# microsoft/M3P

Measured on AMD Instinct MI355X. Metric: pre-train samples/sec (whole node), 12L/768d seq=128+36, higher is better.
Workload: dtype bf16; 1 GPU; cfg2: 12L/768d/12h, 36 regions + 128 tokens, V=250002, 19 MLM targets/seq + ITM BCE, dropout 0.10, adam_inverse_sqrt + clip 5; per_gpu_batch=256, global_batch=256, seq_len=164, parallelism=dp1, prewarm_steps=36

## Files before the change

m3p_amd/csrc/embed.hip:

```cpp
#include "common.hpp"
#include <hip/amd_detail/amd_hip_unsafe_atomics.h>

namespace {

constexpr int EMB_BWD_BLOCKS = 512;

constexpr float kEps = 1e-12f;

template <int NI>
__device__ __forceinline__ void row_ln(const f32x4 (&v)[NI], int nchunk, int lane, float inv_d, float& mu, float& rs) {
  float s = 0.f;
#pragma unroll
  for (int i = 0; i < NI; ++i) s += (v[i][0] + v[i][1]) + (v[i][2] + v[i][3]);
  mu = wave_sum(s) * inv_d;
  float q = 0.f;
#pragma unroll
  for (int i = 0; i < NI; ++i) {
    if (lane + 64 * i < nchunk) {
      const f32x4 t = v[i] - mu;
      q += (t[0] * t[0] + t[1] * t[1]) + (t[2] * t[2] + t[3] * t[3]);
    }
  }
  rs = 1.0f / sqrtf(wave_sum(q) * inv_d + kEps);
}

struct EmbedFwdArgs {
  const int64_t* tok;
  const bf16* emb;
  const float* pos;
  const bf16* img_proj;
  const float* loc;
  const float* w_loc;
  const float* b_loc;
  const float* g_img; const float* be_img;
  const float* g_emb; const float* be_emb;
  const int32_t* totlen;
  bf16* h;
  bf16* z;
  float* mean_emb; float* rstd_emb;
  bf16* e;
  float* mean_img; float* rstd_img;
  int B, T, R, d;
  uint32_t seed_img, seed_emb, thresh24; float inv_keep;
  bf16* img_rows; int img_mode;
};

template <int NI>
__global__ __launch_bounds__(256) void embed_fwd_kernel(EmbedFwdArgs a) {
  const int lane = threadIdx.x & 63;
  const int wave = (blockIdx.x * blockDim.x + threadIdx.x) >> 6;
  const int nwaves = (gridDim.x * blockDim.x) >> 6;
  const int S = a.R + a.T, d = a.d, nchunk = d >> 2;
  const float inv_d = 1.0f / (float)d;
  for (int m = wave; m < a.B * S; m += nwaves) {
    const int b = m / S, s = m - b * S;
    const float mk = (a.img_mode == 1 || s < a.totlen[b]) ? 1.f : 0.f;
    f32x4 v[NI];
    if (s < a.R && a.img_mode == 2) {
#pragma unroll
      for (int i = 0; i < NI; ++i) {
        const int c = lane + 64 * i;
        v[i] = f32x4{0.f, 0.f, 0.f, 0.f};
        if (c < nchunk) v[i] = Vec4<bf16>::load(a.img_rows + ((size_t)b * a.R + s) * d + 4 * c);
      }
    } else if (s < a.R) {
      const int ri = s * a.B + b;
      float lc[5];
#pragma unroll
      for (int k = 0; k < 5; ++k) lc[k] = a.loc[(size_t)ri * 5 + k];
#pragma unroll
      for (int i = 0; i < NI; ++i) {
        const int c = lane + 64 * i;
        v[i] = f32x4{0.f, 0.f, 0.f, 0.f};
        if (c < nchunk) {
          f32x4 t = Vec4<bf16>::load(a.img_proj + (size_t)ri * d + 4 * c) + Vec4<float>::load(a.b_loc + 4 * c);
#pragma unroll
          for (int j = 0; j < 4; ++j) {
            const float* w = a.w_loc + (size_t)(4 * c + j) * 5;
            t[j] += w[0] * lc[0] + w[1] * lc[1] + w[2] * lc[2] + w[3] * lc[3] + w[4] * lc[4];
          }
          t = round_bf16(t);
          Vec4<bf16>::store(a.e + (size_t)ri * d + 4 * c, t);
          v[i] = t;
        }
      }
      float mu, rs;
      row_ln<NI>(v, nchunk, lane, inv_d, mu, rs);
      if (lane == 0) { a.mean_img[ri] = mu; a.rstd_img[ri] = rs; }
#pragma unroll
      for (int i = 0; i < NI; ++i) {
        const int c = lane + 64 * i;
        if (c < nchunk) {
          f32x4 o = (v[i] - mu) * rs * Vec4<float>::load(a.g_img + 4 * c) + Vec4<float>::load(a.be_img + 4 * c);
          if (a.thresh24) {
            const uint32_t base = (uint32_t)ri * (uint32_t)d + 4u * c;
            { bool kp[4]; m3p_keep_even<4>(base, a.seed_img, a.thresh24, kp);
#pragma unroll
          for (int j = 0; j < 4; ++j) o[j] = kp[j] ? o[j] * a.inv_keep : 0.f; }
          }
          v[i] = o;
          if (a.img_mode == 1) Vec4<bf16>::store(a.img_rows + ((size_t)b * a.R + s) * d + 4 * c, o);
        }
      }
      if (a.img_mode == 1) continue;
    } else {
      const int64_t id = a.tok[(size_t)(s - a.R) * a.B + b];
#pragma unroll
      for (int i = 0; i < NI; ++i) {
        const int c = lane + 64 * i;
        v[i] = f32x4{0.f, 0.f, 0.f, 0.f};
        if (c < nchunk) v[i] = Vec4<bf16>::load(a.emb + (size_t)id * d + 4 * c);
      }
    }
#pragma unroll
    for (int i = 0; i < NI; ++i) {
      const int c = lane + 64 * i;
      if (c < nchunk) {
        const f32x4 t = round_bf16((v[i] + Vec4<float>::load(a.pos + (size_t)s * d + 4 * c)) * mk);
        Vec4<bf16>::store(a.z + (size_t)m * d + 4 * c, t);
        v[i] = t;
      }
    }
    float mu, rs;
    row_ln<NI>(v, nchunk, lane, inv_d, mu, rs);
    if (lane == 0) { a.mean_emb[m] = mu; a.rstd_emb[m] = rs; }
#pragma unroll
    for (int i = 0; i < NI; ++i) {
      const int c = lane + 64 * i;
      if (c < nchunk) {
        f32x4 o = (v[i] - mu) * rs * Vec4<float>::load(a.g_emb + 4 * c) + Vec4<float>::load(a.be_emb + 4 * c);
        if (a.thresh24) {
          const uint32_t base = (uint32_t)m * (uint32_t)d + 4u * c;
          { bool kp[4]; m3p_keep_even<4>(base, a.seed_emb, a.thresh24, kp);
#pragma unroll
          for (int j = 0; j < 4; ++j) o[j] = kp[j] ? o[j] * a.inv_keep : 0.f; }
        }
        Vec4<bf16>::store(a.h + (size_t)m * d + 4 * c, o);
      }
    }
  }
}

struct EmbedBwdArgs {
  const bf16* dh;
  const bf16* z; const float* mean_emb; const float* rstd_emb; const float* g_emb;
  const bf16* e; const float* mean_img; const float* rstd_img; const float* g_img;
  const int64_t* tok; const int32_t* totlen; const float* loc;
  bf16* dz;
  bf16* de;
  float* d_g_emb; float* d_be_emb; float* d_pos;
  float* d_emb;
  bf16* d_tok_rows;
  float* d_g_img; float* d_be_img; float* d_b_img; float* d_b_loc; float* d_w_loc;
  int B, T, R, d, pad_index, bsplit;
  uint32_t seed_img, seed_emb, thresh24; float inv_keep;
};

template <int NI>
__device__ __forceinline__ void block_reduce_atomic(float (*red)[NI * 256], const f32x4 (&acc)[NI], float* out, int d,
                                                    int lane, int wib) {
#pragma unroll
  for (int i = 0; i < NI; ++i)
#pragma unroll
    for (int j = 0; j < 4; ++j) red[wib][4 * (lane + 64 * i) + j] = acc[i][j];
  __syncthreads();
  for (int c = threadIdx.x; c < d; c += blockDim.x)
    unsafeAtomicAdd(out + c, (red[0][c] + red[1][c]) + (red[2][c] + red[3][c]));
  __syncthreads();
}

template <int NI>
__global__ __launch_bounds__(256) void embed_bwd_rows_kernel(EmbedBwdArgs a) {
  __shared__ float red[4][NI * 256];
  const int lane = threadIdx.x & 63, wib = threadIdx.x >> 6;
  const int S = a.R + a.T, d = a.d, nchunk = d >> 2;
  const float inv_d = 1.0f / (float)d;
  const int s = blockIdx.x / a.bsplit, part = blockIdx.x - s * a.bsplit;
  f32x4 g[NI], acc_g[NI], acc_b[NI], acc_p[NI];
#pragma unroll
  for (int i = 0; i < NI; ++i) {
    const int c = lane + 64 * i;
    g[i] = f32x4{0.f, 0.f, 0.f, 0.f};
    if (c < nchunk) g[i] = Vec4<float>::load(a.g_emb + 4 * c);
    acc_g[i] = acc_b[i] = acc_p[i] = f32x4{0.f, 0.f, 0.f, 0.f};
  }
  for (int b = part * 4 + wib; b < a.B; b += 4 * a.bsplit) {
    const size_t m = (size_t)b * S + s;
    const float mu = a.mean_emb[m], rs = a.rstd_emb[m];
    const float mk = (s < a.totlen[b]) ? 1.f : 0.f;
    f32x4 dy[NI], xh[NI];
    float s1 = 0.f, s2 = 0.f;
#pragma unroll
    for (int i = 0; i < NI; ++i) {
      const int c = lane + 64 * i;
      dy[i] = xh[i] = f32x4{0.f, 0.f, 0.f, 0.f};
      if (c < nchunk) {
        dy[i] = Vec4<bf16>::load(a.dh + m * d + 4 * c);
        if (a.thresh24) {
          const uint32_t base = (uint32_t)m * (uint32_t)d + 4u * c;
          { bool kp[4]; m3p_keep_even<4>(base, a.seed_emb, a.thresh24, kp);
#pragma unroll
          for (int j = 0; j < 4; ++j) dy[i][j] = kp[j] ? dy[i][j] * a.inv_keep : 0.f; }
        }
        xh[i] = (Vec4<bf16>::load(a.z + m * d + 4 * c) - mu) * rs;
        const f32x4 gd = dy[i] * g[i];
        s1 += (gd[0] + gd[1]) + (gd[2] + gd[3]);
        const f32x4 gx = gd * xh[i];
        s2 += (gx[0] + gx[1]) + (gx[2] + gx[3]);
        acc_g[i] += dy[i] * xh[i];
        acc_b[i] += dy[i];
      }
    }
    const float c1 = wave_sum(s1) * inv_d, c2 = wave_sum(s2) * inv_d;
    int64_t id = -1;
    if (s >= a.R) id = a.tok[(size_t)(s - a.R) * a.B + b];
#pragma unroll
    for (int i = 0; i < NI; ++i) {
      const int c = lane + 64 * i;
      if (c < nchunk) {
        const f32x4 o = (dy[i] * g[i] - c1 - xh[i] * c2) * rs * mk;
        acc_p[i] += o;
        if (s < a.R) {
          Vec4<bf16>::store(a.dz + m * d + 4 * c, o);
        } else {
          *reinterpret_cast<f32x4*>(&red[wib][4 * c]) = o;
        }
      }
    }
    if (s >= a.R && a.d_tok_rows) {
      const bool live = id != a.pad_index && mk != 0.f;
      bf16* dr = a.d_tok_rows + ((size_t)(s - a.R) * a.B + b) * d;
#pragma unroll
      for (int i = 0; i < NI; ++i) {
        const int c = lane + 64 * i;
        if (c < nchunk) {
          f32x4 o = *reinterpret_cast<const f32x4*>(&red[wib][4 * c]);
          if (!live) o = f32x4{0.f, 0.f, 0.f, 0.f};
// ... 19 lines not shown
__global__ __launch_bounds__(256) void embed_bwd_img_kernel(EmbedBwdArgs a) {
  __shared__ float red[4][NI * 256];
  const int lane = threadIdx.x & 63, wib = threadIdx.x >> 6;
  const int S = a.R + a.T, d = a.d, nchunk = d >> 2;
  const float inv_d = 1.0f / (float)d;
  const int r = blockIdx.x / a.bsplit, part = blockIdx.x - r * a.bsplit;
  f32x4 g[NI], acc_g[NI], acc_b[NI], acc_e[NI], acc_w[5][NI];
#pragma unroll
  for (int i = 0; i < NI; ++i) {
    const int c = lane + 64 * i;
    g[i] = f32x4{0.f, 0.f, 0.f, 0.f};
    if (c < nchunk) g[i] = Vec4<float>::load(a.g_img + 4 * c);
    acc_g[i] = acc_b[i] = acc_e[i] = f32x4{0.f, 0.f, 0.f, 0.f};
#pragma unroll
    for (int k = 0; k < 5; ++k) acc_w[k][i] = f32x4{0.f, 0.f, 0.f, 0.f};
  }
  for (int b = part * 4 + wib; b < a.B; b += 4 * a.bsplit) {
    const size_t m = (size_t)b * S + r;
    const size_t ri = (size_t)r * a.B + b;
    const float mu = a.mean_img[ri], rs = a.rstd_img[ri];
    float lc[5];
#pragma unroll
    for (int k = 0; k < 5; ++k) lc[k] = a.loc[ri * 5 + k];
    f32x4 dy[NI], xh[NI];
    float s1 = 0.f, s2 = 0.f;
#pragma unroll
    for (int i = 0; i < NI; ++i) {
      const int c = lane + 64 * i;
      dy[i] = xh[i] = f32x4{0.f, 0.f, 0.f, 0.f};
      if (c < nchunk) {
        dy[i] = Vec4<bf16>::load(a.dz + m * d + 4 * c);
        if (a.thresh24) {
          const uint32_t base = (uint32_t)ri * (uint32_t)d + 4u * c;
          { bool kp[4]; m3p_keep_even<4>(base, a.seed_img, a.thresh24, kp);
#pragma unroll
          for (int j = 0; j < 4; ++j) dy[i][j] = kp[j] ? dy[i][j] * a.inv_keep : 0.f; }
        }
        xh[i] = (Vec4<bf16>::load(a.e + ri * d + 4 * c) - mu) * rs;
        const f32x4 gd = dy[i] * g[i];
        s1 += (gd[0] + gd[1]) + (gd[2] + gd[3]);
        const f32x4 gx = gd * xh[i];
        s2 += (gx[0] + gx[1]) + (gx[2] + gx[3]);
        acc_g[i] += dy[i] * xh[i];
        acc_b[i] += dy[i];
      }
    }
    const float c1 = wave_sum(s1) * inv_d, c2 = wave_sum(s2) * inv_d;
#pragma unroll
    for (int i = 0; i < NI; ++i) {
      const int c = lane + 64 * i;
      if (c < nchunk) {
        const f32x4 ob = round_bf16((dy[i] * g[i] - c1 - xh[i] * c2) * rs);
        Vec4<bf16>::store(a.de + ri * d + 4 * c, ob);
        acc_e[i] += ob;
#pragma unroll
        for (int k = 0; k < 5; ++k) acc_w[k][i] += ob * lc[k];
      }
    }
  }
  block_reduce_atomic<NI>(red, acc_g, a.d_g_img, d, lane, wib);
  block_reduce_atomic<NI>(red, acc_b, a.d_be_img, d, lane, wib);
#pragma unroll
  for (int i = 0; i < NI; ++i)
#pragma unroll
    for (int j = 0; j < 4; ++j) red[wib][4 * (lane + 64 * i) + j] = acc_e[i][j];
  __syncthreads();
  for (int c = threadIdx.x; c < d; c += blockDim.x) {
    const float v = (red[0][c] + red[1][c]) + (red[2][c] + red[3][c]);
    unsafeAtomicAdd(a.d_b_img + c, v);
    unsafeAtomicAdd(a.d_b_loc + c, v);
  }
  __syncthreads();
#pragma unroll
  for (int k = 0; k < 5; ++k) {
#pragma unroll
    for (int i = 0; i < NI; ++i)
#pragma unroll
      for (int j = 0; j < 4; ++j) red[wib][4 * (lane + 64 * i) + j] = acc_w[k][i][j];
    __syncthreads();
    for (int c = threadIdx.x; c < d; c += blockDim.x)
      unsafeAtomicAdd(a.d_w_loc + (size_t)c * 5 + k, (red[0][c] + red[1][c]) + (red[2][c] + red[3][c]));
    __syncthreads();
  }
}

__global__ __launch_bounds__(256) void cast_f32_bf16_kernel(const float* __restrict__ src, bf16* __restrict__ dst, size_t n4) {
  for (size_t i = (size_t)blockIdx.x * blockDim.x + threadIdx.x; i < n4; i += (size_t)gridDim.x * blockDim.x)
    Vec4<bf16>::store(dst + 4 * i, Vec4<float>::load(src + 4 * i));
}

inline int ni_of(int d) { return (d + 255) / 256; }

int launch_embed_fwd(const EmbedFwdArgs& a, void* stream);
}

extern "C" {

int m3p_cast_f32_bf16(const float* src, void* dst, long long n, void* stream) {
  if (n <= 0 || (n % 4) != 0 || ((uintptr_t)src & 15) || ((uintptr_t)dst & 7)) return M3P_EINVAL;
  const size_t n4 = (size_t)n / 4;
  const int blocks = (int)((n4 + 255) / 256 < 4096 ? (n4 + 255) / 256 : 4096);
  hipLaunchKernelGGL(cast_f32_bf16_kernel, dim3(blocks), dim3(256), 0, (hipStream_t)stream, src, (bf16*)dst, n4);
  M3P_CHECK_LAUNCH();
  return M3P_OK;
}

int m3p_embed_assemble_fwd(const int64_t* tok, const void* emb_bf16, const float* pos, const void* img_proj,
                           const float* loc, const float* w_loc, const float* b_loc, const float* g_img,
                           const float* be_img, const float* g_emb, const float* be_emb, const int32_t* totlen,
                           void* h, void* z, float* mean_emb, float* rstd_emb, void* e, float* mean_img,
                           float* rstd_img, int B, int T, int R, int d, uint32_t seed_img, uint32_t seed_emb,
                           uint32_t thresh24, float inv_keep, const void* img_rows, void* stream) {
  if (B <= 0 || T < 0 || R < 0 || d <= 0 || (d % 4) != 0 || d > 1024) return M3P_EINVAL;
  if (img_rows && ((uintptr_t)img_rows & 7)) return M3P_EINVAL;
  EmbedFwdArgs a = {tok, (const bf16*)emb_bf16, pos, (const bf16*)img_proj, loc, w_loc, b_loc, g_img, be_img, g_emb, be_emb,
                    totlen, (bf16*)h, (bf16*)z, mean_emb, rstd_emb, (bf16*)e, mean_img, rstd_img, B, T, R, d,
                    seed_img, seed_emb, thresh24, inv_keep, (bf16*)const_cast<void*>(img_rows), img_rows ? 2 : 0};
  return launch_embed_fwd(a, stream);
}

int m3p_embed_image_rows_fwd(const void* img_proj, const float* loc, const float* w_loc, const float* b_loc,
                             const float* g_img, const float* be_img, void* e, float* mean_img, float* rstd_img,
                             void* img_rows, int B, int R, int d, uint32_t seed_img, uint32_t thresh24, float inv_keep,
                             void* stream) {
  if (B <= 0 || R <= 0 || d <= 0 || (d % 4) != 0 || d > 1024 || !img_rows || ((uintptr_t)img_rows & 7)) return M3P_EINVAL;
  EmbedFwdArgs a = {nullptr, nullptr, nullptr, (const bf16*)img_proj, loc, w_loc, b_loc, g_img, be_img, nullptr, nullptr,
                    nullptr, nullptr, nullptr, nullptr, nullptr, (bf16*)e, mean_img, rstd_img, B, 0, R, d,
                    seed_img, 0u, thresh24, inv_keep, (bf16*)img_rows, 1};
  return launch_embed_fwd(a, stream);
}

}

namespace {
int launch_embed_fwd(const EmbedFwdArgs& a, void* stream) {
  const int B = a.B, T = a.T, R = a.R, d = a.d;
  const int rows = B * (R + T);
  const int blocks = (rows + 3) / 4 < 4096 ? (rows + 3) / 4 : 4096;
  hipStream_t st = (hipStream_t)stream;
  switch (ni_of(d)) {
    case 1: hipLaunchKernelGGL(embed_fwd_kernel<1>, dim3(blocks), dim3(256), 0, st, a); break;
    case 2: hipLaunchKernelGGL(embed_fwd_kernel<2>, dim3(blocks), dim3(256), 0, st, a); break;
    case 3: hipLaunchKernelGGL(embed_fwd_kernel<3>, dim3(blocks), dim3(256), 0, st, a); break;
    default: hipLaunchKernelGGL(embed_fwd_kernel<4>, dim3(blocks), dim3(256), 0, st, a); break;
  }
  M3P_CHECK_LAUNCH();
  return M3P_OK;
}
}

extern "C" {

int m3p_embed_assemble_bwd(const void* dh, const void* z, const float* mean_emb, const float* rstd_emb,
                           const float* g_emb, const void* e, const float* mean_img, const float* rstd_img,
                           const float* g_img, const int64_t* tok, const int32_t* totlen, const float* loc,
                           void* dz_scratch, void* de, float* d_g_emb, float* d_be_emb, float* d_pos, float* d_emb,
                           void* d_tok_rows, float* d_g_img, float* d_be_img, float* d_b_img, float* d_b_loc, float* d_w_loc,
                           int B, int T, int R, int d, int pad_index, uint32_t seed_img, uint32_t seed_emb,
                           uint32_t thresh24, float inv_keep, int phase, void* stream) {
  if (B <= 0 || T < 0 || R < 0 || d <= 0 || (d % 4) != 0 || d > 1024 || phase < 0 || phase > 2) return M3P_EINVAL;
  int bsplit = 1;
  while (bsplit < 16 && (R + T) * bsplit < EMB_BWD_BLOCKS && B / (4 * bsplit) >= 8) bsplit *= 2;
  EmbedBwdArgs a = {(const bf16*)dh, (const bf16*)z, mean_emb, rstd_emb, g_emb, (const bf16*)e, mean_img, rstd_img, g_img,
                    tok, totlen, loc, (bf16*)dz_scratch, (bf16*)de, d_g_emb, d_be_emb, d_pos, d_emb,
                    (bf16*)d_tok_rows, d_g_img, d_be_img, d_b_img, d_b_loc, d_w_loc, B, T, R, d, pad_index, bsplit,
                    seed_img, seed_emb, thresh24, inv_keep};
  hipStream_t st = (hipStream_t)stream;
  const int S = R + T;
#define M3P_EMB_BWD(NI)                                                                              \
  do {                                                                                               \
    if (phase != 2) hipLaunchKernelGGL(embed_bwd_rows_kernel<NI>, dim3(S* bsplit), dim3(256), 0, st, a);             \
    if (R > 0 && phase != 1) hipLaunchKernelGGL(embed_bwd_img_kernel<NI>, dim3(R* bsplit), dim3(256), 0, st, a);   \
  } while (0)
  switch (ni_of(d)) {
    case 1: M3P_EMB_BWD(1); break;
    case 2: M3P_EMB_BWD(2); break;
    case 3: M3P_EMB_BWD(3); break;
    default: M3P_EMB_BWD(4); break;
  }
#undef M3P_EMB_BWD
  M3P_CHECK_LAUNCH();
  return M3P_OK;
}

}
```

m3p_amd/csrc/gemm.hip:

```cpp
#include <mutex>
#include <type_traits>
#include "common.hpp"
#include "../../include/m3p_hip.h"
#include <hip/amd_detail/amd_hip_unsafe_atomics.h>

static int g_variant = 1;
extern "C" void m3p_debug_set_variant(int v) { g_variant = (v == 2 || v == 6) ? v : 1; }

namespace {

constexpr int BK = 64;
constexpr int ROWB = BK * 2;

#define M3P_DSR(dst, addr, off) asm volatile("ds_read_b128 %0, %1 offset:" #off : "=v"(dst) : "v"(addr))
#define M3P_TR(dst, addr, off) asm volatile("ds_read_b64_tr_b16 %0, %1 offset:" #off : "=v"(dst) : "v"(addr))
#define M3P_WAIT_LGKM(N) do { __builtin_amdgcn_sched_barrier(0); asm volatile("s_waitcnt lgkmcnt(" #N ")" ::: "memory"); __builtin_amdgcn_sched_barrier(0); } while (0)
#define M3P_WAIT_VM(N) do { __builtin_amdgcn_sched_barrier(0); asm volatile("s_waitcnt vmcnt(" #N ")" ::: "memory"); __builtin_amdgcn_sched_barrier(0); } while (0)
#define M3P_BAR() do { __builtin_amdgcn_s_barrier(); asm volatile("" ::: "memory"); __builtin_amdgcn_sched_barrier(0); } while (0)

__device__ __forceinline__ int xcd_slot(int nwg) {
  const int per_xcd = nwg >> 3;
  return (blockIdx.x & 7) * per_xcd + (blockIdx.x >> 3);
}
__device__ __forceinline__ int strip_width(int tiles_n, int from, int width) {
// ... 1881 lines not shown
  if (SPLITK) {
    if (wid > 0) {
#pragma unroll
      for (int i = 0; i < MT; ++i) red[wid - 1][i][lane] = acc[i];
    }
    __syncthreads();
    if (wid > 0) return;
#pragma unroll
    for (int i = 0; i < MT; ++i) acc[i] += red[0][i][lane] + red[1][i][lane] + red[2][i][lane];
  }
  f32x4 unused = f32x4{0.f, 0.f, 0.f, 0.f};
#pragma unroll
  for (int i = 0; i < MT; ++i) epilogue_store<EPI>(ep, C, ldc, M, N, i * 16 + fr, n0 + fg * 4, acc[i], unused);
}

template <int EPI, int MT>
int launch_nt_skinny(const bf16* A, int lda, const bf16* W, int ldw, bf16* C, int ldc, int M, int N, int K,
                     const M3PEpilogue& ep, hipStream_t st) {
  if (N <= 8192)
    hipLaunchKernelGGL((gemm_nt_skinny_kernel<EPI, MT, true>), dim3((N + 15) / 16), dim3(256), 0, st, A, lda, W, ldw, C, ldc, M, N, K, ep);
  else
    hipLaunchKernelGGL((gemm_nt_skinny_kernel<EPI, MT, false>), dim3((N + 63) / 64), dim3(256), 0, st, A, lda, W, ldw, C, ldc, M, N, K, ep);
  M3P_CHECK_LAUNCH();
  return M3P_OK;
}

static int hw_cus() {
  static int n = 0;
  if (n == 0) {
    int dev = 0;
    hipDeviceProp_t prop;
    if (hipGetDevice(&dev) == hipSuccess && hipGetDeviceProperties(&prop, dev) == hipSuccess) n = prop.multiProcessorCount;
    if (n <= 0) n = 256;
    n -= n % 8;
    if (n <= 0) n = 8;
  }
  return n;
}
static int g_persistent_grid = 0;
static int num_cus() {
  const int hw = hw_cus();
  return (g_persistent_grid > 0 && g_persistent_grid < hw) ? g_persistent_grid : hw;
}
static int persistent_grid(int ntiles) {
  const int grid = num_cus();
  return ntiles < grid ? (ntiles + 7) / 8 * 8 : grid;
}
template <auto Kern>
int set_max_lds(size_t lds) {
  static bool done = false;
  if (!done) {
    hipError_t e = hipFuncSetAttribute((const void*)Kern, hipFuncAttributeMaxDynamicSharedMemorySize, (int)lds);
    if (e != hipSuccess) return (int)e;
    done = true;
  }
  return M3P_OK;
}

static int* g_tq_pool = nullptr;
static int g_tq_slots = 0, g_tq_next = 0;
static hipStream_t g_tq_stream = nullptr;
static bool g_tq_bound = false;
static std::mutex g_tq_mu;
static int* tq_acquire(hipStream_t st, hipError_t* err) {
  *err = hipSuccess;
  std::lock_guard<std::mutex> lk(g_tq_mu);
  if (!g_tq_pool) return nullptr;
  if (!g_tq_bound) { g_tq_stream = st; g_tq_bound = true; }
  if (st != g_tq_stream) return nullptr;
  if (g_tq_next == g_tq_slots) {
    *err = hipMemsetAsync(g_tq_pool, 0, (size_t)g_tq_slots * 8 * sizeof(int), st);
    if (*err != hipSuccess) return nullptr;
    g_tq_next = 0;
  }
  return g_tq_pool + 8 * g_tq_next++;
}

constexpr int W4_MIN_K = 2048;
static bool tq_enabled() {
  std::lock_guard<std::mutex> lk(g_tq_mu);
  return g_tq_pool != nullptr;
}

static int nt_plan(int epi, int M, int N, int K, int* queue) {
  if (queue) *queue = 0;
  const bool whole = M >= 1024 && (M % 256) == 0 && (N % 256) == 0 && N >= 512 && (K % 64) == 0;
  if (epi == M3P_EPI_MULQ || epi == M3P_EPI_BIAS_GELUQ || epi == M3P_EPI_BIAS_LSE) return whole ? M3P_KERN_NT_W8 : M3P_EINVAL;
  const bool mul_epi = epi == M3P_EPI_DGELU || epi == M3P_EPI_MUL;
  if (M <= 128 && (K % 128) == 0 && !mul_epi) return M3P_KERN_NT_SKINNY;
  const bool deep = N >= 512 && 2LL * N * K <= (64LL << 20) && epi != M3P_EPI_DGELU;
  const bool armed = tq_enabled();
  const bool w4_first = g_variant == 1 && deep && K >= W4_MIN_K && epi != M3P_EPI_MUL && !armed;
  if (whole && g_variant != 2 && !w4_first) {
    const int ntiles = (M / 256) * (N / 256);
    if (queue) *queue = (!mul_epi && armed && ntiles > persistent_grid(ntiles) && K >= 8 * BK) ? 1 : 0;
    return M3P_KERN_NT_W8;
  }
  if (M >= 1024 && (M % 256) == 0 && (N % 256) == 0 && (g_variant == 2 || (g_variant == 1 && deep)))
    return M3P_KERN_NT_W4;
  if (M >= 1024) return M3P_KERN_NT_RING;
  return M3P_KERN_NT_128;
}

template <int EPI>
int launch_nt(const bf16* A, int lda, const bf16* W, int ldw, bf16* C, int ldc, int M, int N, int K,
              const M3PEpilogue& ep, hipStream_t st) {
  int want_queue = 0;
  const int plan = nt_plan(EPI, M, N, K, &want_queue);
  if (plan == M3P_KERN_NT_SKINNY) {
    if constexpr (EPI != M3P_EPI_DGELU && EPI != M3P_EPI_MUL) {
      if (M <= 16) return launch_nt_skinny<EPI, 1>(A, lda, W, ldw, C, ldc, M, N, K, ep, st);
      if (M <= 32) return launch_nt_skinny<EPI, 2>(A, lda, W, ldw, C, ldc, M, N, K, ep, st);
      if (M <= 64) return launch_nt_skinny<EPI, 4>(A, lda, W, ldw, C, ldc, M, N, K, ep, st);
      return launch_nt_skinny<EPI, 8>(A, lda, W, ldw, C, ldc, M, N, K, ep, st);
    }
  }
  if (plan == M3P_KERN_NT_W8) {
    const int tiles_m = M / 256, tiles_n = N / 256;
    const size_t lds = 2 * 512 * ROWB + (EPI == M3P_EPI_DGELU ? GELU_TAB_N * sizeof(float) : 0) +
                       ((EPI == M3P_EPI_DGELU || EPI == M3P_EPI_MUL) ? 8 * 2048 : 8 * 4096);
    constexpr auto kern = gemm_nt_w8_kernel<EPI>;
    if (int rc = set_max_lds<kern>(lds)) return rc;
    const int grid = persistent_grid(tiles_m * tiles_n);
    constexpr bool kQueueOk = !(EPI == M3P_EPI_DGELU || EPI == M3P_EPI_MUL);
    int* ctr = nullptr;
    if (kQueueOk && want_queue) {
      hipError_t e;
      ctr = tq_acquire(st, &e);
      if (e != hipSuccess) return (int)e;
    }
    if constexpr (kQueueOk) if (ctr) {
      constexpr auto kern_d = gemm_nt_w8_kernel<EPI, true>;
      if (int rc = set_max_lds<kern_d>(lds)) return rc;
      hipLaunchKernelGGL(kern_d, dim3(grid), dim3(512), lds, st, A, lda, W, ldw, C, ldc, M, N, K, ep, tiles_m, tiles_n, ctr);
      M3P_CHECK_LAUNCH();
      return M3P_OK;
    }
    hipLaunchKernelGGL(kern, dim3(grid), dim3(512), lds, st, A, lda, W, ldw, C, ldc, M, N, K, ep, tiles_m, tiles_n, ctr);
    M3P_CHECK_LAUNCH();
    return M3P_OK;
  }
  if (plan == M3P_KERN_NT_W4) {
    constexpr int BM = 256, BN = 256;
    const int tiles_m = (M + BM - 1) / BM, tiles_n = (N + BN - 1) / BN;
    const size_t lds = 2 * (BM + BN) * 128 + 4 * EP_HALF;
    const bool rows = (EPI == M3P_EPI_BIAS_DROP_RES && ep.rng_rows != nullptr);
    constexpr auto kern_rows = gemm_nt_w4_kernel<(EPI == M3P_EPI_BIAS_DROP_RES ? M3P_EPI_DROP_RES_ROWS : EPI)>, kern_plain = gemm_nt_w4_kernel<EPI>;
    if (int rc = rows ? set_max_lds<kern_rows>(lds) : set_max_lds<kern_plain>(lds)) return rc;
    auto kern = rows ? kern_rows : kern_plain;
    const int grid = persistent_grid(tiles_m * tiles_n);
    const long long wbytes = 2LL * N * K, abytes = 2LL * M * K;
    const int m_fast = (wbytes > (64LL << 20) && abytes < wbytes) ? 1 : 0;
    hipLaunchKernelGGL(kern, dim3(grid), dim3(256), lds, st, A, lda, W, ldw, C, ldc, M, N, K, ep, tiles_m, tiles_n, m_fast);
    M3P_CHECK_LAUNCH();
    return M3P_OK;
  }
  if (plan == M3P_KERN_NT_RING) {
    constexpr int BM = 256, BN = 128;
    const int tiles_m = (M + BM - 1) / BM, tiles_n = (N + BN - 1) / BN;
    const size_t lds = 3 * (BM + BN) * ROWB + (EPI == M3P_EPI_DGELU ? GELU_TAB_N * sizeof(float) : 0);
    constexpr auto kern = gemm_nt_ring_kernel<EPI>;
    if (int rc = set_max_lds<kern>(lds)) return rc;
    const int grid = persistent_grid(tiles_m * tiles_n);
    hipLaunchKernelGGL(kern, dim3(grid), dim3(512), lds, st, A, lda, W, ldw, C, ldc, M, N, K, ep, tiles_m, tiles_n);
    M3P_CHECK_LAUNCH();
    return M3P_OK;
  }
  constexpr int BM = 128, BN = 128;
  const int tiles_m = (M + BM - 1) / BM, tiles_n = (N + BN - 1) / BN;
  const size_t lds = 2 * (BM + BN) * ROWB;
  constexpr auto kern = gemm_nt_kernel<BM, BN, EPI>;
  if (int rc = set_max_lds<kern>(lds)) return rc;
  hipLaunchKernelGGL(kern, dim3(tiles_m * tiles_n), dim3(256), lds, st, A, lda, W, ldw, C, ldc, M, N, K, ep,
                     tiles_m, tiles_n);
// ... 722 lines not shown
```

m3p_amd/csrc/glue.hip:

```cpp
#include "common.hpp"

namespace {

__global__ __launch_bounds__(256)
void seq_masks_kernel(const long long* __restrict__ len_a, const long long* __restrict__ len_b, int B, int S,
                      int* __restrict__ totlen, uint8_t* __restrict__ rowmask) {
  const int b = blockIdx.x;
  const int n = (int)(len_a[b] + (len_b ? len_b[b] : 0));
  if (threadIdx.x == 0) totlen[b] = n;
  for (int s = threadIdx.x; s < S; s += blockDim.x) rowmask[(size_t)b * S + s] = (s < n) ? 1 : 0;
}

__global__ __launch_bounds__(1024)
void mask_to_rows_kernel(const uint8_t* __restrict__ mask, int n_mask, int inner, long long s0, long long s1,
                         long long soff, int d, int* __restrict__ rows, int n_rows) {
  __shared__ int wsum[16];
  __shared__ int total_sh;
  const int tid = threadIdx.x, lane = tid & 63, w = tid >> 6;
  const int per = (n_mask + 1023) / 1024;
  const int lo = min(tid * per, n_mask), hi = min(lo + per, n_mask);
  int cnt = 0;
  for (int i = lo; i < hi; ++i) cnt += mask[i] ? 1 : 0;
  int inc = cnt;
#pragma unroll
  for (int o = 1; o < 64; o <<= 1) {
    const int v = __shfl_up(inc, o, 64);
    if (lane >= o) inc += v;
  }
  if (lane == 63) wsum[w] = inc;
  __syncthreads();
  if (tid == 0) {
    int run = 0;
    for (int i = 0; i < 16; ++i) { const int v = wsum[i]; wsum[i] = run; run += v; }
    total_sh = run;
  }
  __syncthreads();
  int pos = wsum[w] + inc - cnt;
  for (int i = lo; i < hi; ++i) {
    if (mask[i]) {
      if (pos < n_rows) {
        const int t = i / inner, b = i - t * inner;
        rows[pos] = (int)((soff + t * s0 + b * s1) / d);
      }
      ++pos;
    }
  }
  for (int k = total_sh + tid; k < n_rows; k += 1024) rows[k] = 0;
}

__global__ __launch_bounds__(256)
void cast_rows_kernel(const float* __restrict__ in, long long s0, long long s1, int n1, int cols,
                      bf16* __restrict__ out, long long nrows) {
  const int cpr = cols >> 2;
  const long long total = nrows * cpr;
  for (long long i = (long long)blockIdx.x * blockDim.x + threadIdx.x; i < total; i += (long long)gridDim.x * blockDim.x) {
    const long long row = i / cpr;
    const int c = (int)(i - row * cpr) * 4;
    const long long i0 = row / n1, i1 = row - i0 * n1;
    const f32x4 v = *reinterpret_cast<const f32x4*>(in + i0 * s0 + i1 * s1 + c);
    *reinterpret_cast<bf16x4*>(out + row * cols + c) = bf16x4{(bf16)v[0], (bf16)v[1], (bf16)v[2], (bf16)v[3]};
  }
}

template <typename TI>
__global__ __launch_bounds__(256)
void scale_to_bf16_kernel(const TI* __restrict__ in, const float* __restrict__ g, bf16* __restrict__ out, long long n4) {
  const float s = g[0];
  for (long long i = (long long)blockIdx.x * blockDim.x + threadIdx.x; i < n4; i += (long long)gridDim.x * blockDim.x) {
    f32x4 v = Vec4<TI>::load(in + 4 * i);
    v *= s;
    Vec4<bf16>::store(out + 4 * i, v);
  }
}

__global__ __launch_bounds__(256)
void axpy_dev_kernel(float* __restrict__ dst, const float* __restrict__ src, const float* __restrict__ g, long long n) {
  const float s = g[0];
  for (long long i = (long long)blockIdx.x * blockDim.x + threadIdx.x; i < n; i += (long long)gridDim.x * blockDim.x)
    dst[i] += s * src[i];
}

__device__ __forceinline__ float softplus_f(float x) {
  return fmaxf(x, 0.f) + log1pf(__expf(-fabsf(x)));
}

__global__ __launch_bounds__(256)
void itm_loss_kernel(const float* __restrict__ scores, const long long* __restrict__ pos, int G, int n, float w_ce,
                     float w_bce, float* __restrict__ loss, float* __restrict__ dscores) {
  __shared__ float red[4];
  float acc = 0.f;
  const float inv_g = 1.f / (float)G, inv_all = 1.f / ((float)G * (float)n);
  for (int g = threadIdx.x; g < G; g += blockDim.x) {
    const float* s = scores + (size_t)g * n;
    const long long p64 = pos[g];
    const bool bad = p64 < 0 || p64 >= n;
    const int p = bad ? 0 : (int)p64;
    float lse = 0.f;
    if (w_ce != 0.f) {
      float mx = -INFINITY;
      for (int j = 0; j < n; ++j) mx = fmaxf(mx, s[j]);
      float se = 0.f;
      for (int j = 0; j < n; ++j) se += __expf(s[j] - mx);
      lse = mx + __logf(se);
    }
    float l = bad ? __builtin_nanf("") : 0.f;
    if (w_ce != 0.f) l += w_ce * inv_g * (lse - s[p]);
    for (int j = 0; j < n; ++j) {
      const float y = (j == p) ? 1.f : 0.f;
      float d = 0.f;
      if (w_ce != 0.f) d += w_ce * inv_g * (__expf(s[j] - lse) - y);
      if (w_bce != 0.f) {
        l += w_bce * inv_all * (softplus_f(s[j]) - y * s[j]);
        d += w_bce * inv_all * (1.f / (1.f + __expf(-s[j])) - y);
      }
      dscores[(size_t)g * n + j] = d;
    }
    acc += l;
  }
  acc = wave_sum(acc);
  if ((threadIdx.x & 63) == 0) red[threadIdx.x >> 6] = acc;
  __syncthreads();
  if (threadIdx.x == 0) loss[0] = red[0] + red[1] + red[2] + red[3];
}

int grid_for(long long work, int per_block) {
  long long g = (work + per_block - 1) / per_block;
  return (int)(g < 1 ? 1 : (g > 2048 ? 2048 : g));
}
// ... 63 lines not shown
```

Before: 8018 sequences/s.

## Add 8-wide embedding backward kernels, hot-token dedup, ring GEMM for underfilled shapes, vector mask scan

```diff
diff --git a/m3p_amd/csrc/embed.hip b/m3p_amd/csrc/embed.hip
--- a/m3p_amd/csrc/embed.hip
+++ b/m3p_amd/csrc/embed.hip
@@ -4,6 +4,7 @@
 namespace {
 
 constexpr int EMB_BWD_BLOCKS = 512;
+constexpr int EMB_IMG_BLOCKS = 256;
 
 constexpr float kEps = 1e-12f;
 
@@ -153,6 +154,7 @@
   bf16* d_tok_rows;
   float* d_g_img; float* d_be_img; float* d_b_img; float* d_b_loc; float* d_w_loc;
   int B, T, R, d, pad_index, bsplit;
+  int bsplit_img;
   uint32_t seed_img, seed_emb, thresh24; float inv_keep;
 };
 
@@ -338,6 +340,317 @@
       unsafeAtomicAdd(a.d_w_loc + (size_t)c * 5 + k, (red[0][c] + red[1][c]) + (red[2][c] + red[3][c]));
     __syncthreads();
   }
+}
+
+template <bool A16>
+__device__ __forceinline__ bf16x8 emb_load8(const bf16* p) {
+  if constexpr (A16) return *reinterpret_cast<const bf16x8*>(p);
+  const bf16x4 lo = *reinterpret_cast<const bf16x4*>(p), hi = *reinterpret_cast<const bf16x4*>(p + 4);
+  return __builtin_shufflevector(lo, hi, 0, 1, 2, 3, 4, 5, 6, 7);
+}
+template <bool A16>
+__device__ __forceinline__ void emb_store8(bf16* p, bf16x8 v) {
+  if constexpr (A16) {
+    *reinterpret_cast<bf16x8*>(p) = v;
+  } else {
+    *reinterpret_cast<bf16x4*>(p) = __builtin_shufflevector(v, v, 0, 1, 2, 3);
+    *reinterpret_cast<bf16x4*>(p + 4) = __builtin_shufflevector(v, v, 4, 5, 6, 7);
+  }
+}
+__device__ __forceinline__ void load_f8(const float* p, float (&o)[8]) {
+  const f32x4 lo = Vec4<float>::load(p), hi = Vec4<float>::load(p + 4);
+#pragma unroll
+  for (int e = 0; e < 4; ++e) { o[e] = lo[e]; o[4 + e] = hi[e]; }
+}
+__device__ __forceinline__ float sum8(const float (&t)[8]) {
+  return ((t[0] + t[1]) + (t[2] + t[3])) + ((t[4] + t[5]) + (t[6] + t[7]));
+}
+__device__ __forceinline__ void keep8(uint32_t base, uint32_t seed, uint32_t thresh24, float inv_keep, float (&o)[8]) {
+  bool kp[8];
+  m3p_keep_even<8>(base, seed, thresh24, kp);
+#pragma unroll
+  for (int e = 0; e < 8; ++e) o[e] = kp[e] ? o[e] * inv_keep : 0.f;
+}
+
+template <int NI>
+__device__ __forceinline__ void block_reduce_atomic8(float (*red)[NI * 512], const float (&acc)[NI][8], float* out, int d,
+                                                     int lane, int wib) {
+#pragma unroll
+  for (int i = 0; i < NI; ++i)
+#pragma unroll
+    for (int e = 0; e < 8; ++e) red[wib][8 * (lane + 64 * i) + e] = acc[i][e];
+  __syncthreads();
+  for (int c = threadIdx.x; c < d; c += blockDim.x)
+    unsafeAtomicAdd(out + c, (red[0][c] + red[1][c]) + (red[2][c] + red[3][c]));
+  __syncthreads();
+}
+
+template <int NI, bool A16>
+__global__ __launch_bounds__(256, 3) void embed_bwd_rows_w_kernel(EmbedBwdArgs a) {
+  __shared__ float red[4][NI * 512];
+  const int lane = threadIdx.x & 63, wib = threadIdx.x >> 6;
+  const int S = a.R + a.T, d = a.d;
+  const float inv_d = 1.0f / (float)d;
+  const int s = blockIdx.x / a.bsplit, part = blockIdx.x - s * a.bsplit;
+  int col[NI];
+  bool on[NI];
+  __shared__ float gs[NI * 512];
+  __shared__ float hot[4][NI * 512];
+  __shared__ long long cand[64];
+  __shared__ long long hot_sh;
+  for (int c = threadIdx.x; c < d; c += blockDim.x) gs[c] = a.g_emb[c];
+  for (int c = threadIdx.x; c < 4 * NI * 512; c += blockDim.x) (&hot[0][0])[c] = 0.f;
+  const bool scatter = s >= a.R && a.d_tok_rows == nullptr;
+  if (scatter && threadIdx.x < 64) {
+    const int bb = part * 4 + (lane & 3) + 4 * a.bsplit * (lane >> 2);
+    long long w = -1;
+    if (bb < a.B) {
+      w = a.tok[(size_t)(s - a.R) * a.B + bb];
+      if (w == a.pad_index) w = -1;
+    }
+    cand[lane] = w;
+  }
+  __syncthreads();
+  if (scatter && threadIdx.x < 64) {
+    const long long mine = cand[lane];
+    int cnt = 0;
+    for (int u = 0; u < 64; ++u) cnt += (cand[u] == mine) ? 1 : 0;
+    int key = (mine < 0 ? 0 : cnt) * 64 + (63 - lane);
+#pragma unroll
+    for (int o = 32; o > 0; o >>= 1) key = max(key, __shfl_xor(key, o, 64));
+    if (lane == 0) hot_sh = (key >> 6) >= 2 ? cand[63 - (key & 63)] : -1;
+  }
+  __syncthreads();
+  const long long hot_id = scatter ? hot_sh : -1;
+  float acc_g[NI][8], acc_b[NI][8], acc_p[NI][8];
+#pragma unroll
+  for (int i = 0; i < NI; ++i) {
+    col[i] = 8 * (lane + 64 * i);
+    on[i] = col[i] < d;
+#pragma unroll
+    for (int e = 0; e < 8; ++e) acc_g[i][e] = acc_b[i][e] = acc_p[i][e] = 0.f;
+  }
+  bf16x8 rdy[NI], rz[NI];
+#pragma unroll
+  for (int i = 0; i < NI; ++i) rdy[i] = rz[i] = bf16x8{};
+  float mu_n = 0.f, rs_n = 0.f;
+  int tl_n = 0;
+  int64_t id_n = -1;
+  auto request = [&](int bb) {
+    if (bb >= a.B) return;
+    const size_t m = (size_t)bb * S + s;
+#pragma unroll
+    for (int i = 0; i < NI; ++i) {
+      if (on[i]) {
+        rdy[i] = emb_load8<A16>(a.dh + m * d + col[i]);
+        rz[i] = emb_load8<A16>(a.z + m * d + col[i]);
+      }
+    }
+    mu_n = a.mean_emb[m]; rs_n = a.rstd_emb[m]; tl_n = a.totlen[bb];
+    if (s >= a.R) id_n = a.tok[(size_t)(s - a.R) * a.B + bb];
+  };
+  const int step = 4 * a.bsplit;
+  int b = part * 4 + wib;
+  request(b);
+  for (; b < a.B; b += step) {
+    const size_t m = (size_t)b * S + s;
+    const float mu = mu_n, rs = rs_n;
+    const float mk = (s < tl_n) ? 1.f : 0.f;
+    const int64_t id = id_n;
+    float dy[NI][8], xh[NI][8];
+#pragma unroll
+    for (int i = 0; i < NI; ++i)
+#pragma unroll
+      for (int e = 0; e < 8; ++e) { dy[i][e] = on[i] ? (float)rdy[i][e] : 0.f; xh[i][e] = on[i] ? (float)rz[i][e] : 0.f; }
+    request(b + step);
+    float s1 = 0.f, s2 = 0.f;
+#pragma unroll
+    for (int i = 0; i < NI; ++i) {
+      if (on[i]) {
+        if (a.thresh24) keep8((uint32_t)m * (uint32_t)d + (uint32_t)col[i], a.seed_emb, a.thresh24, a.inv_keep, dy[i]);
+        float g[8], gd[8], gx[8];
+        load_f8(&gs[col[i]], g);
+#pragma unroll
+        for (int e = 0; e < 8; ++e) {
+          xh[i][e] = (xh[i][e] - mu) * rs;
+          gd[e] = dy[i][e] * g[e];
+          gx[e] = gd[e] * xh[i][e];
+          acc_g[i][e] += dy[i][e] * xh[i][e];
+          acc_b[i][e] += dy[i][e];
+        }
+        s1 += sum8(gd);
+        s2 += sum8(gx);
+      } else {
+#pragma unroll
+        for (int e = 0; e < 8; ++e) xh[i][e] = 0.f;
+      }
+    }
+    const float c1 = wave_sum(s1) * inv_d, c2 = wave_sum(s2) * inv_d;
+    const bool tok_row = s >= a.R;
+    const bool live = tok_row && id != a.pad_index && mk != 0.f;
+#pragma unroll
+    for (int i = 0; i < NI; ++i) {
+      if (on[i]) {
+        float o[8], g[8];
+        load_f8(&gs[col[i]], g);
+        bf16x8 ob;
+#pragma unroll
+        for (int e = 0; e < 8; ++e) {
+          o[e] = (dy[i][e] * g[e] - c1 - xh[i][e] * c2) * rs * mk;
+          acc_p[i][e] += o[e];
+          ob[e] = (bf16)o[e];
+        }
+        if (!tok_row) {
+          emb_store8<A16>(a.dz + m * d + col[i], ob);
+        } else if (a.d_tok_rows) {
+          if (!live) ob = bf16x8{};
+          emb_store8<A16>(a.d_tok_rows + ((size_t)(s - a.R) * a.B + b) * d + col[i], ob);
+        } else if (live && id == hot_id) {
+          *reinterpret_cast<f32x4*>(&hot[wib][col[i]]) += f32x4{o[0], o[1], o[2], o[3]};
+          *reinterpret_cast<f32x4*>(&hot[wib][col[i] + 4]) += f32x4{o[4], o[5], o[6], o[7]};
+        } else {
+          *reinterpret_cast<f32x4*>(&red[wib][col[i]]) = f32x4{o[0], o[1], o[2], o[3]};
+          *reinterpret_cast<f32x4*>(&red[wib][col[i] + 4]) = f32x4{o[4], o[5], o[6], o[7]};
+        }
+      }
+    }
+    if (live && !a.d_tok_rows && id != hot_id) {
+      float* de = a.d_emb + (size_t)id * d;
+      __builtin_amdgcn_wave_barrier();
+#pragma unroll
+      for (int k = 0; k < 8 * NI; ++k) {
+        const int e = lane + 64 * k;
+        if (e < d) unsafeAtomicAdd(de + e, red[wib][e]);
+      }
+      __builtin_amdgcn_wave_barrier();
+    }
+  }
+  __syncthreads();
+  block_reduce_atomic8<NI>(red, acc_g, a.d_g_emb, d, lane, wib);
+  block_reduce_atomic8<NI>(red, acc_b, a.d_be_emb, d, lane, wib);
+  block_reduce_atomic8<NI>(red, acc_p, a.d_pos + (size_t)s * d, d, lane, wib);
+  if (hot_id >= 0) {
+    float* de = a.d_emb + (size_t)hot_id * d;
+    for (int c = threadIdx.x; c < d; c += blockDim.x)
+      unsafeAtomicAdd(de + c, (hot[0][c] + hot[1][c]) + (hot[2][c] + hot[3][c]));
+  }
+}
+
+template <int NI, bool A16>
+__global__ __launch_bounds__(256) void embed_bwd_img_w_kernel(EmbedBwdArgs a) {
+  __shared__ float red[4][NI * 512];
+  __shared__ float wsum[NI * 512 * 5];
+  const int lane = threadIdx.x & 63, wib = threadIdx.x >> 6;
+  const int S = a.R + a.T, d = a.d;
+  const float inv_d = 1.0f / (float)d;
+  const int r = blockIdx.x / a.bsplit_img, part = blockIdx.x - r * a.bsplit_img;
+  int col[NI];
+  bool on[NI];
+  float g[NI][8], acc_g[NI][8], acc_b[NI][8], acc_e[NI][8], acc_w[5][NI][8];
+#pragma unroll
+  for (int i = 0; i < NI; ++i) {
+    col[i] = 8 * (lane + 64 * i);
+    on[i] = col[i] < d;
+#pragma unroll
+    for (int e = 0; e < 8; ++e) {
+      g[i][e] = acc_g[i][e] = acc_b[i][e] = acc_e[i][e] = 0.f;
+#pragma unroll
+      for (int k = 0; k < 5; ++k) acc_w[k][i][e] = 0.f;
+    }
+    if (on[i]) load_f8(a.g_img + col[i], g[i]);
+  }
+  bf16x8 rdz[NI], re[NI];
+#pragma unroll
+  for (int i = 0; i < NI; ++i) rdz[i] = re[i] = bf16x8{};
+  float mu_n = 0.f, rs_n = 0.f, lc_n[5] = {0.f, 0.f, 0.f, 0.f, 0.f};
+  auto request = [&](int bb) {
+    if (bb >= a.B) return;
+    const size_t m = (size_t)bb * S + r, ri = (size_t)r * a.B + bb;
+#pragma unroll
+    for (int i = 0; i < NI; ++i) {
+      if (on[i]) {
+        rdz[i] = emb_load8<A16>(a.dz + m * d + col[i]);
+        re[i] = emb_load8<A16>(a.e + ri * d + col[i]);
+      }
+    }
+    mu_n = a.mean_img[ri]; rs_n = a.rstd_img[ri];
+#pragma unroll
+    for (int k = 0; k < 5; ++k) lc_n[k] = a.loc[ri * 5 + k];
+  };
+  const int step = 4 * a.bsplit_img;
+  int b = part * 4 + wib;
+  request(b);
+  for (; b < a.B; b += step) {
+    const size_t ri = (size_t)r * a.B + b;
+    const float mu = mu_n, rs = rs_n;
+    float lc[5];
+#pragma unroll
+    for (int k = 0; k < 5; ++k) lc[k] = lc_n[k];
+    float dy[NI][8], xh[NI][8];
+#pragma unroll
+    for (int i = 0; i < NI; ++i)
+#pragma unroll
+      for (int e = 0; e < 8; ++e) { dy[i][e] = on[i] ? (float)rdz[i][e] : 0.f; xh[i][e] = on[i] ? (float)re[i][e] : 0.f; }
+    request(b + step);
+    float s1 = 0.f, s2 = 0.f;
+#pragma unroll
+    for (int i = 0; i < NI; ++i) {
+      if (on[i]) {
+        if (a.thresh24) keep8((uint32_t)ri * (uint32_t)d + (uint32_t)col[i], a.seed_img, a.thresh24, a.inv_keep, dy[i]);
+        float gd[8], gx[8];
+#pragma unroll
+        for (int e = 0; e < 8; ++e) {
+          xh[i][e] = (xh[i][e] - mu) * rs;
+          gd[e] = dy[i][e] * g[i][e];
+          gx[e] = gd[e] * xh[i][e];
+          acc_g[i][e] += dy[i][e] * xh[i][e];
+          acc_b[i][e] += dy[i][e];
+        }
+        s1 += sum8(gd);
+        s2 += sum8(gx);
+      }
+    }
+    const float c1 = wave_sum(s1) * inv_d, c2 = wave_sum(s2) * inv_d;
+#pragma unroll
+    for (int i = 0; i < NI; ++i) {
+      if (on[i]) {
+        bf16x8 ob;
+#pragma unroll
+        for (int e = 0; e < 8; ++e) {
+          ob[e] = (bf16)((dy[i][e] * g[i][e] - c1 - xh[i][e] * c2) * rs);
+          const float of = (float)ob[e];
+          acc_e[i][e] += of;
+#pragma unroll
+          for (int k = 0; k < 5; ++k) acc_w[k][i][e] += of * lc[k];
+        }
+        emb_store8<A16>(a.de + ri * d + col[i], ob);
+      }
+    }
+  }
+  block_reduce_atomic8<NI>(red, acc_g, a.d_g_img, d, lane, wib);
+  block_reduce_atomic8<NI>(red, acc_b, a.d_be_img, d, lane, wib);
+#pragma unroll
+  for (int i = 0; i < NI; ++i)
+#pragma unroll
+    for (int e = 0; e < 8; ++e) red[wib][8 * (lane + 64 * i) + e] = acc_e[i][e];
+  __syncthreads();
+  for (int c = threadIdx.x; c < d; c += blockDim.x) {
+    const float v = (red[0][c] + red[1][c]) + (red[2][c] + red[3][c]);
+    unsafeAtomicAdd(a.d_b_img + c, v);
+    unsafeAtomicAdd(a.d_b_loc + c, v);
+  }
+  __syncthreads();
+#pragma unroll
+  for (int k = 0; k < 5; ++k) {
+#pragma unroll
+    for (int i = 0; i < NI; ++i)
+#pragma unroll
+      for (int e = 0; e < 8; ++e) red[wib][8 * (lane + 64 * i) + e] = acc_w[k][i][e];
+    __syncthreads();
+    for (int c = threadIdx.x; c < d; c += blockDim.x) wsum[c * 5 + k] = (red[0][c] + red[1][c]) + (red[2][c] + red[3][c]);
+    __syncthreads();
+  }
+  for (int j = threadIdx.x; j < 5 * d; j += blockDim.x) unsafeAtomicAdd(a.d_w_loc + j, wsum[j]);
 }
 
 __global__ __launch_bounds__(256) void cast_f32_bf16_kernel(const float* __restrict__ src, bf16* __restrict__ dst, size_t n4) {
@@ -419,10 +732,30 @@
   while (bsplit < 16 && (R + T) * bsplit < EMB_BWD_BLOCKS && B / (4 * bsplit) >= 8) bsplit *= 2;
   EmbedBwdArgs a = {(const bf16*)dh, (const bf16*)z, mean_emb, rstd_emb, g_emb, (const bf16*)e, mean_img, rstd_img, g_img,
                     tok, totlen, loc, (bf16*)dz_scratch, (bf16*)de, d_g_emb, d_be_emb, d_pos, d_emb,
-                    (bf16*)d_tok_rows, d_g_img, d_be_img, d_b_img, d_b_loc, d_w_loc, B, T, R, d, pad_index, bsplit,
+                    (bf16*)d_tok_rows, d_g_img, d_be_img, d_b_img, d_b_loc, d_w_loc, B, T, R, d, pad_index, bsplit, 1,
                     seed_img, seed_emb, thresh24, inv_keep};
   hipStream_t st = (hipStream_t)stream;
   const int S = R + T;
+  if ((d % 8) == 0) {
+    while (a.bsplit_img < 64 && R * a.bsplit_img < EMB_IMG_BLOCKS && B / (8 * a.bsplit_img) >= 4) a.bsplit_img *= 2;
+    const bool a16_rows = !(((uintptr_t)dh | (uintptr_t)z | (uintptr_t)dz_scratch | (uintptr_t)d_tok_rows) & 15);
+    const bool a16_img = !(((uintptr_t)dz_scratch | (uintptr_t)e | (uintptr_t)de) & 15);
+#define M3P_EMB_BWD_W(NI)                                                                                                     \
+  do {                                                                                                                        \
+    if (phase != 2) {                                                                                                         \
+      if (a16_rows) hipLaunchKernelGGL((embed_bwd_rows_w_kernel<NI, true>), dim3(S * bsplit), dim3(256), 0, st, a);           \
+      else hipLaunchKernelGGL((embed_bwd_rows_w_kernel<NI, false>), dim3(S * bsplit), dim3(256), 0, st, a);                   \
+    }                                                                                                                         \
+    if (R > 0 && phase != 1) {                                                                                                \
+      if (a16_img) hipLaunchKernelGGL((embed_bwd_img_w_kernel<NI, true>), dim3(R * a.bsplit_img), dim3(256), 0, st, a);       \
+      else hipLaunchKernelGGL((embed_bwd_img_w_kernel<NI, false>), dim3(R * a.bsplit_img), dim3(256), 0, st, a);              \
+    }                                                                                                                         \
+  } while (0)
+    if (d <= 512) M3P_EMB_BWD_W(1); else M3P_EMB_BWD_W(2);
+#undef M3P_EMB_BWD_W
+    M3P_CHECK_LAUNCH();
+    return M3P_OK;
+  }
 #define M3P_EMB_BWD(NI)                                                                              \
   do {                                                                                               \
     if (phase != 2) hipLaunchKernelGGL(embed_bwd_rows_kernel<NI>, dim3(S* bsplit), dim3(256), 0, st, a);             \
diff --git a/m3p_amd/csrc/gemm.hip b/m3p_amd/csrc/gemm.hip
--- a/m3p_amd/csrc/gemm.hip
+++ b/m3p_amd/csrc/gemm.hip
@@ -1987,6 +1987,11 @@
   return g_tq_pool != nullptr;
 }
 
+static bool nt_underfilled(int M, int N) {
+  const int tiles_m = M / 256;
+  return 2LL * tiles_m * (N / 256) <= num_cus() && (tiles_m & (tiles_m - 1)) != 0;
+}
+
 static int nt_plan(int epi, int M, int N, int K, int* queue) {
   if (queue) *queue = 0;
   const bool whole = M >= 1024 && (M % 256) == 0 && (N % 256) == 0 && N >= 512 && (K % 64) == 0;
@@ -1995,6 +2000,7 @@
   if (M <= 128 && (K % 128) == 0 && !mul_epi) return M3P_KERN_NT_SKINNY;
   const bool deep = N >= 512 && 2LL * N * K <= (64LL << 20) && epi != M3P_EPI_DGELU;
   const bool armed = tq_enabled();
+  if (whole && g_variant == 1 && !armed && !mul_epi && nt_underfilled(M, N)) return M3P_KERN_NT_RING;
   const bool w4_first = g_variant == 1 && deep && K >= W4_MIN_K && epi != M3P_EPI_MUL && !armed;
   if (whole && g_variant != 2 && !w4_first) {
     const int ntiles = (M / 256) * (N / 256);
diff --git a/m3p_amd/csrc/glue.hip b/m3p_amd/csrc/glue.hip
--- a/m3p_amd/csrc/glue.hip
+++ b/m3p_amd/csrc/glue.hip
@@ -19,8 +19,25 @@
   const int tid = threadIdx.x, lane = tid & 63, w = tid >> 6;
   const int per = (n_mask + 1023) / 1024;
   const int lo = min(tid * per, n_mask), hi = min(lo + per, n_mask);
+  const bool wide = (per & 15) == 0 && per <= 64 && (n_mask & 15) == 0 && ((uintptr_t)mask & 15) == 0;
+  uint32_t wv[16];
   int cnt = 0;
-  for (int i = lo; i < hi; ++i) cnt += mask[i] ? 1 : 0;
+  if (wide) {
+#pragma unroll
+    for (int q = 0; q < 4; ++q) {
+      uint4 t = make_uint4(0u, 0u, 0u, 0u);
+      if (lo + 16 * q < hi) t = *reinterpret_cast<const uint4*>(mask + lo + 16 * q);
+      wv[4 * q] = t.x; wv[4 * q + 1] = t.y; wv[4 * q + 2] = t.z; wv[4 * q + 3] = t.w;
+    }
+#pragma unroll
+    for (int k = 0; k < 16; ++k) {
+      uint32_t x = wv[k];
+      x |= x >> 4; x |= x >> 2; x |= x >> 1;
+      cnt += __popc(x & 0x01010101u);
+    }
+  } else {
+    for (int i = lo; i < hi; ++i) cnt += mask[i] ? 1 : 0;
+  }
   int inc = cnt;
 #pragma unroll
   for (int o = 1; o < 64; o <<= 1) {
@@ -36,14 +53,24 @@
   }
   __syncthreads();
   int pos = wsum[w] + inc - cnt;
-  for (int i = lo; i < hi; ++i) {
-    if (mask[i]) {
-      if (pos < n_rows) {
-        const int t = i / inner, b = i - t * inner;
-        rows[pos] = (int)((soff + t * s0 + b * s1) / d);
-      }
-      ++pos;
-    }
+  auto emit = [&](int i) {
+    if (pos < n_rows) {
+      const int t = i / inner, b = i - t * inner;
+      rows[pos] = (int)((soff + t * s0 + b * s1) / d);
+    }
+    ++pos;
+  };
+  if (wide) {
+#pragma unroll
+    for (int k = 0; k < 16; ++k) {
+      if (wv[k] == 0u) continue;
+#pragma unroll
+      for (int j = 0; j < 4; ++j)
+        if ((wv[k] >> (8 * j)) & 0xFFu) emit(lo + 4 * k + j);
+    }
+  } else {
+    for (int i = lo; i < hi; ++i)
+      if (mask[i]) emit(i);
   }
   for (int k = total_sh + tid; k < n_rows; k += 1024) rows[k] = 0;
 }
```

Result: no change. 8087 sequences/s, median of 6 (+0.9%).
